# semihkacmaz/CoNFiLD

Measured on AMD Instinct MI355X. Metric: generated fields/sec (256-step sample + CNF decode), Case4 latent, 1/2/4/8 GPU, higher is better.
Workload: dtype f32

## Files before the change

### confild_amd/_lib.py

```python
from __future__ import annotations

import ctypes as C
import os
import threading

_HERE = os.path.dirname(os.path.abspath(__file__))
LIB_PATH = os.path.join(_HERE, "lib", "libconfild_hip.so")
if os.environ.get("CFD_LIB"):
    LIB_PATH = os.path.join(_HERE, "lib", os.path.basename(os.environ["CFD_LIB"]))

_lock = threading.Lock()
_lib = None

c_f32p = C.POINTER(C.c_float)
c_i64p = C.POINTER(C.c_int64)


class CfdError(RuntimeError):
    pass


class UNetCfg(C.Structure):
    _fields_ = [("image_size", C.c_int), ("in_channels", C.c_int), ("model_channels", C.c_int),
                ("out_channels", C.c_int), ("num_res_blocks", C.c_int), ("n_mult", C.c_int),
# ... 35 lines not shown
                                     C.c_void_p, C.c_size_t, C.c_void_p]),
    "cfd_unet_set_tape_mode": (C.c_int, [C.c_void_p, C.c_int]),
    "cfd_sched_create": (C.c_int, [C.c_void_p, C.c_int, C.c_int, C.POINTER(C.c_void_p)]),
    "cfd_sched_destroy": (None, [C.c_void_p]),
    "cfd_sched_step": (C.c_int, [C.c_void_p, C.c_int, C.c_int, C.c_void_p, C.c_void_p, C.c_void_p, C.c_void_p,
                                 C.c_uint64, C.c_uint64, C.c_uint64, C.c_void_p, C.c_void_p, C.c_int64, C.c_int,
                                 C.c_void_p]),
    "cfd_sched_step_known": (C.c_int, [C.c_void_p, C.c_int, C.c_int, C.c_void_p, C.c_void_p, C.c_void_p, C.c_void_p,
                                       C.c_uint64, C.c_uint64, C.c_uint64, C.c_void_p, C.c_void_p, C.c_int64,
                                       C.c_int, C.c_void_p, C.c_int64, C.c_void_p, C.c_int64, C.c_void_p,
                                       C.c_void_p, C.c_uint64, C.c_void_p]),
    "cfd_sched_step_jump": (C.c_int, [C.c_void_p, C.c_int, C.c_int, C.c_void_p, C.c_void_p, C.c_void_p, C.c_void_p,
                                      C.c_uint64, C.c_uint64, C.c_uint64, C.c_void_p, C.c_void_p, C.c_int64,
                                      C.c_int, C.c_void_p, C.c_int64, C.c_void_p, C.c_int64, C.c_void_p,
                                      C.c_void_p, C.c_uint64, C.c_float, C.c_float, C.c_void_p, C.c_uint64,
                                      C.c_void_p]),
    "cfd_sampler_set_jumps": (C.c_int, [C.c_void_p, C.c_void_p]),
    "cfd_sampler_set_known": (C.c_int, [C.c_void_p, C.c_void_p, C.c_int64, C.c_void_p, C.c_int64, C.c_void_p,
                                        C.c_void_p]),
    "cfd_sampler_captures": (C.c_int, [C.c_void_p, C.POINTER(C.c_uint64)]),
    "cfd_dps_latent_residual_workspace_bytes": (C.c_int, [C.c_int64, C.c_int, C.POINTER(C.c_size_t)]),
    "cfd_dps_latent_residual": (C.c_int, [C.c_void_p, C.c_int, C.c_void_p, C.c_void_p, C.c_void_p, C.c_void_p,
                                          C.c_int64, C.c_void_p, C.c_int64, C.c_void_p, C.c_void_p, C.c_void_p,
                                          C.c_int64, C.c_int, C.c_void_p, C.c_size_t, C.c_void_p]),
    "cfd_sampler_create": (C.c_int, [C.c_void_p, C.c_void_p, C.c_int, C.c_int, C.c_int, C.c_int64, C.c_int,
                                     C.c_void_p, C.c_void_p, C.c_int, C.c_int, C.POINTER(C.c_void_p)]),
    "cfd_sampler_destroy": (None, [C.c_void_p]),
    "cfd_sampler_run": (C.c_int, [C.c_void_p, C.c_void_p, C.c_void_p, C.c_int, C.c_int, C.c_uint64, C.c_uint64,
                                  C.c_void_p]),
    "cfd_randn": (C.c_int, [C.c_void_p, C.c_int64, C.c_uint64, C.c_uint64, C.c_uint64, C.c_void_p]),
    "cfd_sine_probe": (C.c_int, [C.c_void_p, C.c_void_p, C.c_int64, C.c_int, C.c_void_p]),
    "cfd_latent_denorm": (C.c_int, [C.c_void_p, C.c_void_p, C.c_int64, C.c_void_p, C.c_void_p, C.c_int64,
                                    C.c_void_p]),
    "cfd_dps_residual": (C.c_int, [C.c_void_p, C.c_int64, C.c_void_p, C.c_void_p, C.c_void_p, C.c_int64, C.c_int,
                                   C.c_void_p]),
    "cfd_dps_latent_grad": (C.c_int, [C.c_void_p, C.c_int, C.c_void_p, C.c_void_p, C.c_void_p, C.c_void_p,
                                      C.c_void_p, C.c_void_p, C.c_int64, C.c_void_p, C.c_void_p, C.c_int64, C.c_int,
                                      C.c_void_p]),
    "cfd_dps_update": (C.c_int, [C.c_void_p, C.c_void_p, C.c_void_p, C.c_float, C.c_void_p, C.c_int64,
                                 C.c_void_p]),
    "cfd_dps_update_known": (C.c_int, [C.c_void_p, C.c_void_p, C.c_void_p, C.c_float, C.c_void_p, C.c_void_p,
                                       C.c_int64, C.c_int, C.c_void_p, C.c_int64, C.c_void_p, C.c_int64, C.c_void_p,
                                       C.c_void_p, C.c_uint64, C.c_uint64, C.c_uint64, C.c_void_p]),
    "cfd_siren_create": (C.c_int, [C.POINTER(SirenCfg), C.c_int, C.POINTER(C.c_void_p)]),
    "cfd_siren_destroy": (None, [C.c_void_p]),
    "cfd_siren_num_params": (C.c_int, [C.c_void_p, C.POINTER(C.c_int)]),
    "cfd_siren_param_info": (C.c_int, [C.c_void_p, C.c_int, C.POINTER(C.c_char_p), C.POINTER(C.c_int),
                                       C.c_int64 * 4]),
    "cfd_siren_set_param": (C.c_int, [C.c_void_p, C.c_char_p, C.c_void_p, C.c_size_t]),
    "cfd_siren_ready": (C.c_int, [C.c_void_p]),
    "cfd_siren_workspace_bytes": (C.c_int, [C.c_void_p, C.c_int, C.POINTER(C.c_size_t)]),
    "cfd_siren_set_compute": (C.c_int, [C.c_void_p, C.c_int]),
    "cfd_siren_get_compute": (C.c_int, [C.c_void_p, C.POINTER(C.c_int)]),
    "cfd_siren_forward": (C.c_int, [C.c_void_p, C.c_void_p, C.c_int64, C.c_void_p, C.c_int, C.c_void_p,
                                    C.c_void_p, C.c_void_p, C.c_void_p, C.c_int64, C.c_void_p, C.c_void_p,
                                    C.c_size_t, C.c_void_p]),
    "cfd_siren_vjp_workspace_bytes": (C.c_int, [C.c_void_p, C.c_int64, C.c_int, C.POINTER(C.c_size_t)]),
    "cfd_siren_tape_forward": (C.c_int, [C.c_void_p, C.c_void_p, C.c_int64, C.c_void_p, C.c_int, C.c_void_p,
                                         C.c_void_p, C.c_void_p, C.c_void_p, C.c_int64, C.c_void_p, C.c_void_p,
                                         C.c_size_t, C.c_void_p]),
    "cfd_siren_tape_vjp": (C.c_int, [C.c_void_p, C.c_void_p, C.c_int64, C.c_int, C.c_void_p, C.c_void_p,
                                     C.c_int64, C.c_void_p, C.c_void_p, C.c_size_t, C.c_void_p]),
    "cfd_siren_dense_plan": (C.c_int, [C.POINTER(SirenCfg), C.c_int64, C.c_int, C.c_size_t, C.c_int, C.c_int,
                                       C.POINTER(C.c_size_t), C.POINTER(C.c_int64), C.POINTER(C.c_int)]),
    "cfd_siren_dense_workspace_bytes": (C.c_int, [C.c_void_p, C.c_int64, C.c_int, C.c_size_t,
                                                  C.POINTER(C.c_size_t)]),
    "cfd_siren_dense_grad": (C.c_int, [C.c_void_p, C.c_void_p, C.c_int64, C.c_void_p, C.c_int, C.c_int, C.c_void_p,
                                       C.c_void_p, C.c_void_p, C.c_void_p, C.c_int64, C.c_void_p, C.c_int,
                                       C.c_void_p, C.c_int, C.c_void_p, C.c_void_p, C.c_void_p, C.c_size_t,
                                       C.c_size_t, C.c_void_p]),
    "cfd_siren_dense_set_form": (C.c_int, [C.c_void_p, C.c_int, C.c_int]),
    "cfd_siren_train_workspace_bytes": (C.c_int, [C.c_void_p, C.c_int64, C.c_int, C.POINTER(C.c_size_t)]),
    "cfd_siren_train_grad": (C.c_int, [C.c_void_p, C.c_void_p, C.c_int64, C.c_void_p, C.c_void_p, C.c_int,
                                       C.c_void_p, C.c_float, C.c_void_p, C.c_void_p, C.c_void_p, C.c_void_p,
                                       C.c_size_t, C.c_void_p]),
    "cfd_unet_param_grad_workspace_bytes": (C.c_int, [C.c_void_p, C.c_int, C.POINTER(C.c_size_t)]),
    "cfd_unet_param_grad": (C.c_int, [C.c_void_p, C.c_void_p, C.c_void_p, C.c_int, C.c_void_p, C.c_size_t,
                                      C.c_void_p, C.c_void_p, C.c_size_t, C.c_void_p]),
    "cfd_eps_mse": (C.c_int, [C.c_void_p, C.c_void_p, C.c_void_p, C.c_void_p, C.c_int64, C.c_int, C.c_float,
                              C.c_void_p, C.c_void_p]),
    "cfd_ema_update": (C.c_int, [C.c_void_p, C.c_void_p, C.c_int64, C.c_double, C.c_void_p]),
    "cfd_q_sample": (C.c_int, [C.c_void_p, C.c_void_p, C.c_void_p, C.c_void_p, C.c_void_p, C.c_int64, C.c_int,
                               C.c_void_p]),
    "cfd_adam_step": (C.c_int, [C.c_void_p, C.c_void_p, C.c_void_p, C.c_void_p, C.c_int64, C.c_double, C.c_double,
                                C.c_double, C.c_double, C.c_double, C.c_int64, C.c_void_p]),
}

EXPORTS = tuple(_SIGS)


def load(path: str = LIB_PATH):
    global _lib
    with _lock:
        if _lib is not None:
            return _lib
        if not os.path.exists(path):
            raise CfdError(f"{path} is missing: build it with `python -c 'import __graft_entry__ as g; g.build()'` "
                           "(or `make -C confild_amd/csrc`)")
        lib = C.CDLL(path)
        for name, (res, args) in _SIGS.items():
            if os.environ.get("CFD_LIB") and not hasattr(lib, name):
                continue
            fn = getattr(lib, name)
            fn.restype = res
            fn.argtypes = args
        _lib = lib
# ... 27 lines not shown
```

### confild_amd/csrc/capi.cpp

```cpp
#include <string>

#include "common.hpp"

namespace cfd {
static thread_local std::string g_last_error;
void set_error(const std::string& msg) { g_last_error = msg; }
}

extern "C" const char* cfd_last_error(void) { return cfd::g_last_error.c_str(); }

extern "C" const char* cfd_version(void) {
    return "libconfild_hip gfx950 r6 (split-f16 / bf16 / fp32 MFMA; native sampler graphs; planned batch; CU-range streams; split-f16 DPS tape; key-chunked attention)";
}
```

### confild_amd/csrc/siren.hpp

```cpp
#pragma once
#include <string>
#include <type_traits>
#include <utility>
#include <vector>

#include "common.hpp"

namespace cfd {

template <int N, class F, int... I>
__device__ __forceinline__ void static_for_impl(F&& f, std::integer_sequence<int, I...>) {
    (f(std::integral_constant<int, I>{}), ...);
}
template <int N, class F>
__device__ __forceinline__ void static_for(F&& f) {
    static_for_impl<N>(f, std::make_integer_sequence<int, N>{});
}

struct SirenArgs {
    const float* w0;
    const float* wimg;
    const float* wout;
    const float* bout;
    const float* film;
    const float* coords;
    const float* xmax;
    const float* xmin;
    const float* ymax;
    const float* ymin;
    float* out;
    const float* wscale;
    const float* wimg_rev;
    const float* wrev;
    int64_t N;
    int64_t ystride;
    int64_t b0;
    int d, c, nh;
    float w0f;
    unsigned long long* stamps;
};
struct SirenTapeArgs {
    const float* w0;
    const float* wimg;
    const float* wimg_t;
    const float* wout;
    const float* bout;
    const float* film;
    const float* coords;
    const float* xmax;
    const float* xmin;
    const float* ymax;
    const float* ymin;
    float* u;
    float* delta;
    float* out;
    const float* gout;
    const float* wimg16;
    const float* wimg16t;
    const float* wscale;
    int64_t P;
    int64_t ystride;
    int Ns, d, c, nh;
    float w0f;
};
unsigned long long* stamps_buf();

template <int NB, int WAVES>
__device__ __forceinline__ void siren_issue_block(const float* __restrict__ wimg, int J, float* dst,
                                                  int wave, int lane) {
    constexpr int BLK = NB * 256;
    const float* src = wimg + (int64_t)__builtin_amdgcn_readfirstlane(J) * BLK;
    for (int piece = wave; piece < NB; piece += WAVES) {
        __builtin_amdgcn_global_load_lds((const void*)(src + piece * 256 + lane * 4),
                                         (__attribute__((address_space(3))) void*)(dst + piece * 256),
                                         16, 0, 0);
    }
}

template <int NB, int WAVES>
__device__ __forceinline__ void siren_issue_block_u(const float* __restrict__ wimg, int J, float* dst,
                                                    int wave, int lane) {
    static_assert(NB % WAVES == 0, "whole pieces per wave");
    constexpr int BLK = NB * 256;
    const float* src = wimg + (int64_t)__builtin_amdgcn_readfirstlane(J) * BLK;
    static_for<NB / WAVES>([&](auto mc) {
        constexpr int m = decltype(mc)::value;
        const int piece = wave + m * WAVES;
        __builtin_amdgcn_global_load_lds((const void*)(src + piece * 256 + lane * 4),
                                         (__attribute__((address_space(3))) void*)(dst + piece * 256), 16, 0, 0);
    });
}

bool siren_split_supported(int NB);
void launch_siren_split(int NB, SirenArgs a, int b, hipStream_t st);
bool siren_split32_supported(int H, int nh);
void launch_siren_split32(int H, SirenArgs a, int b, hipStream_t st);
bool tape_split_supported(int NB);
void launch_tape_split(int NB, const SirenTapeArgs& a, bool bwd, hipStream_t st);
void launch_tape_split_sum(int NB, const SirenTapeArgs& a, int rows, hipStream_t st);

struct SirenParam {
    std::string key;
    std::vector<int64_t> shape;
    bool set = false;
};

}

struct cfd_siren {
    cfd_siren_cfg cfg;
    int device = 0;
    int NB = 0;
    std::vector<cfd::SirenParam> params;
    float* w0 = nullptr;
    float* fbias = nullptr;
    float* V = nullptr;
    float* wimg = nullptr;
    float* wout = nullptr;
    float* bout = nullptr;
    float* wimg_t = nullptr;
    float* wimg16 = nullptr;
    float* wimg16t = nullptr;
    float* wscale = nullptr;
    float* wimg32 = nullptr;
    float* wimg32r = nullptr;
    float* wrev = nullptr;
    int compute = CFD_SIREN_SPLIT_F16;
    int dense_bwd = CFD_DENSE_BWD_SUM;
    int dense_compute = CFD_DENSE_COMPUTE_AUTO;
};

namespace cfd {

int gemm_splits(int K);
void launch_gemm_f32(bool bt, const float* A, int lda, const float* B, int ldb, const float* bias, float* C, int ldc,
                     int M, int N, int K, hipStream_t st, float* part = nullptr);
void film_vectors(const cfd_siren* h, const float* latents, int b, float* film, hipStream_t st);

}
```

### confild_amd/csrc/siren_split.hip

```cpp
#include <cstdint>
#include <cstdlib>
#include <algorithm>

#include "siren.hpp"

typedef _Float16 h8 __attribute__((ext_vector_type(8)));
typedef _Float16 h2 __attribute__((ext_vector_type(2)));
typedef float f2 __attribute__((ext_vector_type(2)));
typedef unsigned u2 __attribute__((ext_vector_type(2)));
typedef unsigned u4 __attribute__((ext_vector_type(4)));

namespace cfd {

struct Frag {
    u4 v;
    __device__ __forceinline__ h8 h() const { return __builtin_bit_cast(h8, v); }
};

__device__ __forceinline__ unsigned pk_f16(float a, float b) {
    return __builtin_bit_cast(unsigned, __builtin_convertvector((f2){a, b}, h2));
}

__device__ __forceinline__ void split8(const float (&x0)[4], const float (&x1)[4], Frag& hi, Frag& lo) {
    unsigned hw[4], lw[4];
#pragma unroll
    for (int w = 0; w < 4; ++w) {
        const float a = w < 2 ? x0[2 * w] : x1[2 * w - 4];
        const float b = w < 2 ? x0[2 * w + 1] : x1[2 * w - 3];
        hw[w] = pk_f16(a, b);
        const f2 hf = __builtin_convertvector(__builtin_bit_cast(h2, hw[w]), f2);
        lw[w] = pk_f16(a - hf.x, b - hf.y);
    }
    hi.v = (u4){hw[0], hw[1], hw[2], hw[3]};
    lo.v = (u4){lw[0], lw[1], lw[2], lw[3]};
    asm volatile("" : "+v"(hi.v), "+v"(lo.v));
}

__device__ __forceinline__ f2 sin2_cw(f2 x) {
    const f2 magic = {12582912.0f, 12582912.0f};
    const f2 t = __builtin_elementwise_fma(x, (f2){0.318309886183790671538f, 0.318309886183790671538f}, magic);
    const f2 q = t - magic;
    f2 r = __builtin_elementwise_fma(q, (f2){-3.140625f, -3.140625f}, x);
    r = __builtin_elementwise_fma(q, (f2){-0.0009670257568359375f, -0.0009670257568359375f}, r);
    r = __builtin_elementwise_fma(q, (f2){-6.2771141529083251953e-07f, -6.2771141529083251953e-07f}, r);
    r = __builtin_elementwise_fma(q, (f2){-1.2154201256553420762e-10f, -1.2154201256553420762e-10f}, r);
    const f2 s = r * r;
    f2 u = (f2){2.6083159809786593541503e-06f, 2.6083159809786593541503e-06f};
    u = __builtin_elementwise_fma(u, s, (f2){-0.0001981069071916863322258f, -0.0001981069071916863322258f});
    u = __builtin_elementwise_fma(u, s, (f2){0.00833307858556509017944336f, 0.00833307858556509017944336f});
    u = __builtin_elementwise_fma(u, s, (f2){-0.166666597127914428710938f, -0.166666597127914428710938f});
    const f2 y = __builtin_elementwise_fma(s, u * r, r);
    const u2 sg = __builtin_bit_cast(u2, t) << 31;
    return __builtin_bit_cast(f2, __builtin_bit_cast(u2, y) + sg);
}

// ... 251 lines not shown
        });
        sines(prev);
        epilogue(std::integral_constant<int, NB - 1>{});
        static_for<NQ>([&](auto qc) {
            constexpr int q = decltype(qc)::value;
#pragma unroll
            for (int c = 0; c < CG; ++c) {
                BH[c][q] = NH[c][q];
                BL[c][q] = NL[c][q];
            }
        });
    }

#pragma unroll
    for (int c = 0; c < CG; ++c) {
        float ov[4];
#pragma unroll
        for (int oc = 0; oc < 4; ++oc) {
            float sum = o[c][oc];
            sum += __shfl_xor(sum, 16);
            sum += __shfl_xor(sum, 32);
            ov[oc] = oc < p.c ? sum + p.bout[oc] : 0.f;
        }
        const int64_t n = n0 + 16 * c;
        if (n < p.N && g < p.c) {
            float v = g == 0 ? ov[0] : g == 1 ? ov[1] : g == 2 ? ov[2] : ov[3];
            if (p.ymax) {
                const int64_t yi = n * p.ystride + g;
                const float hi = p.ymax[yi], lo = p.ymin[yi];
                v = (v + 1.0f) / 2.0f * (hi - lo) + lo;
            }
            p.out[(b * p.N + n) * p.c + g] = v;
        }
    }
}

typedef float f16v __attribute__((ext_vector_type(16)));

__device__ __forceinline__ void split2_mix(float a, float b, unsigned& hi, unsigned& lo) {
    hi = pk_f16(a, b);
    asm("v_fma_mixlo_f16 %0, %1, 1.0, -%2 op_sel_hi:[0,0,1]" : "=&v"(lo) : "v"(a), "v"(hi));
    asm("v_fma_mixhi_f16 %0, %1, 1.0, -%2 op_sel:[0,0,1] op_sel_hi:[0,0,1]" : "+v"(lo) : "v"(b), "v"(hi));
}

__device__ __forceinline__ void split_chunk(const float (&x)[16], int e, Frag& hi, Frag& lo) {
    unsigned hw[4], lw[4];
#pragma unroll
    for (int w = 0; w < 4; ++w) split2_mix(x[8 * e + 2 * w], x[8 * e + 2 * w + 1], hw[w], lw[w]);
    hi.v = (u4){hw[0], hw[1], hw[2], hw[3]};
    lo.v = (u4){lw[0], lw[1], lw[2], lw[3]};
    asm volatile("" : "+v"(hi.v), "+v"(lo.v));
}

template <int NB2, int EXP = 0, int HWSIN = 0>
__global__ __launch_bounds__(256, 1) void siren_split32(SirenArgs p) {
    constexpr int NK = 2 * NB2;
    constexpr int H = 32 * NB2;
    constexpr int BLK = NK * 512;
    constexpr int WAVES = 4, TILE = 128;
    constexpr int NPC = 2 * NK;
    constexpr int PPW = NPC / WAVES;
    constexpr int NKS = NK >= 18 ? 16 : NK - 2;
    extern __shared__ __attribute__((aligned(16))) float smem[];
    const int nh = p.nh;
    float* wbuf = smem;
    float* film = smem + 2 * BLK;
    float* w0s = film + (nh + 1) * H;
    float* wos = w0s + 4 * H;

    const int lane = threadIdx.x & 63;
    const int wave = __builtin_amdgcn_readfirstlane(threadIdx.x >> 6);
    const int h = lane >> 5;
    const int64_t b = p.b0 + blockIdx.y;
    const int64_t n = (int64_t)blockIdx.x * TILE + wave * 32 + (lane & 31);
    CFD_DASSERT(p.d >= 1 && p.d <= 4 && p.c >= 1 && p.c <= 4 && nh >= 1);
#ifdef CFD_STAMPS
    const bool stamped = blockIdx.x % 61 == 0;
    if (stamped) CFD_STAMP(p.stamps, 5, (unsigned)blockIdx.y, 0);
    __builtin_amdgcn_s_waitcnt(0xC07F);
#endif

    {
        const float* fsrc = p.film + b * (int64_t)(nh + 1) * H;
        const int nf = (nh + 1) * H;
        for (int i = threadIdx.x * 4; i < nf; i += 64 * WAVES * 4) {
            const int layer = i / H;
            const float sc = layer == 0 ? 1.0f : HWSIN >= 3 ? p.wrev[layer - 1] : p.wscale[layer - 1];
            *(f4*)(film + i) = *(const f4*)(fsrc + i) * sc;
        }
    }
    for (int f = threadIdx.x; f < H; f += 64 * WAVES) {
        f4 w = {0.f, 0.f, 0.f, 0.f};
        for (int k = 0; k < p.d; ++k) w[k] = p.w0[f * p.d + k];
        *(f4*)(w0s + 4 * f) = w;
    }
    for (int i = threadIdx.x; i < 4 * H; i += 64 * WAVES) wos[i] = i < p.c * H ? p.wout[i] : 0.f;
    float cn[4];
    {
        const int64_t nc = n < p.N ? n : p.N - 1;
#pragma unroll
        for (int k = 0; k < 4; ++k) {
            float v = 0.f;
            if (k < p.d) {
                v = p.coords[nc * p.d + k];
                if (p.xmax) v = (v - p.xmin[k]) / (p.xmax[k] - p.xmin[k]) * 2.0f - 1.0f;
            }
            cn[k] = v;
        }
    }
    __syncthreads();
    const int nblocks = nh * NB2;
    const __amdgpu_buffer_rsrc_t wrsrc =
        __builtin_amdgcn_make_buffer_rsrc((void*)p.wimg, 0, nblocks * (BLK * 4), 0x00020000);
    siren_issue_block<NPC, WAVES>(p.wimg, 0, wbuf, wave, lane);

    Frag BH[NK], BL[NK], NH[NK], NL[NK];
    float o[4] = {0.f, 0.f, 0.f, 0.f};

    static_for<NB2>([&](auto Jc) {
        constexpr int J = decltype(Jc)::value;
        float x[16];
#pragma unroll
        for (int qq = 0; qq < 4; ++qq) {
            const f4 fv = *(const f4*)(film + 32 * J + 8 * qq + 4 * h);
#pragma unroll
            for (int r = 0; r < 4; ++r) {
                const f4 w = *(const f4*)(w0s + 4 * (32 * J + 8 * qq + 4 * h + r));
                float a = cn[0] * w[0];
#pragma unroll
                for (int k = 1; k < 4; ++k)
                    if (k < p.d) a = fmaf(cn[k], w[k], a);
                x[4 * qq + r] = hidden_sine<HWSIN >= 2 ? 2 : HWSIN>(p.w0f * (a + fv[r]));
            }
        }
        split_chunk(x, 0, NH[2 * J], NL[2 * J]);
        split_chunk(x, 1, NH[2 * J + 1], NL[2 * J + 1]);
    });

    static_assert(NB2 % 2 == 0, "static ring slots need an even block count");
    int J = 0;
    f16v prev;
    float mprev = 0.f;
    float x[16];
    for (int layer = 1; layer <= nh; ++layer) {
        const bool last = layer == nh;
        const float m = HWSIN >= 3 ? p.wrev[nh + layer - 1] : p.w0f / p.wscale[layer - 1];
        auto outsum = [&](int jp, int e) __attribute__((always_inline)) {
            const int f = 32 * jp + 8 * e + 4 * h;
#pragma unroll
            for (int oc = 0; oc < 4; ++oc) {
                const f4 w = *(const f4*)(wos + oc * H + f);
#pragma unroll
                for (int r = 0; r < 4; ++r) o[oc] = fmaf(w[r], x[4 * e + r], o[oc]);
            }
        };
        static_for<NB2>([&](auto jc) {
            constexpr int j = decltype(jc)::value;
            constexpr int jp = j == 0 ? NB2 - 1 : j - 1;
            const float me = j == 0 ? mprev : m;
            const bool live = j > 0 || layer > 1;
            float* nxt = wbuf + ((j & 1) ^ 1) * BLK;
            const float* wb = wbuf + (j & 1) * BLK;
            const int soff = __builtin_amdgcn_readfirstlane(min(J + 1, nblocks - 1)) * (BLK * 4);
            f16v a;
#pragma unroll
            for (int qq = 0; qq < 4; ++qq) {
                const f4 f = *(const f4*)(film + layer * H + 32 * j + 8 * qq + 4 * h);
#pragma unroll
                for (int r = 0; r < 4; ++r) a[4 * qq + r] = f[r];
            }
            h8 FH = *(const h8*)(wb + lane * 4);
            h8 FL = *(const h8*)(wb + 256 + lane * 4);
            static_for<NK>([&](auto kc) {
                constexpr int k = decltype(kc)::value;
                h8 FH1 = FH, FL1 = FL;
                if constexpr (k + 1 < NK && !(EXP & 4)) {
                    FH1 = *(const h8*)(wb + (k + 1) * 512 + lane * 4);
                    FL1 = *(const h8*)(wb + (k + 1) * 512 + 256 + lane * 4);
                }
                if constexpr (k < PPW && !(EXP & 1)) {
                    const int piece = wave + WAVES * k;
                    __builtin_amdgcn_raw_ptr_buffer_load_lds(
                        wrsrc, (__attribute__((address_space(3))) void*)(nxt + piece * 256), 16, lane * 16,
                        soff + piece * 1024, 0, 0);
                }
                if constexpr (j == 0) {
                    a = __builtin_amdgcn_mfma_f32_32x32x16_f16(FL, NH[k].h(), a, 0, 0, 0);
                    a = __builtin_amdgcn_mfma_f32_32x32x16_f16(FH, NL[k].h(), a, 0, 0, 0);
                    a = __builtin_amdgcn_mfma_f32_32x32x16_f16(FH, NH[k].h(), a, 0, 0, 0);
                    BH[k] = NH[k];
                    BL[k] = NL[k];
                    asm volatile("" : "+a"(BH[k].v), "+a"(BL[k].v));
                } else {
                    a = __builtin_amdgcn_mfma_f32_32x32x16_f16(FL, BH[k].h(), a, 0, 0, 0);
                    a = __builtin_amdgcn_mfma_f32_32x32x16_f16(FH, BL[k].h(), a, 0, 0, 0);
                    a = __builtin_amdgcn_mfma_f32_32x32x16_f16(FH, BH[k].h(), a, 0, 0, 0);
                }
                if constexpr (k < NKS) {
#pragma unroll
                    for (int v = 16 * k / NKS; v < 16 * (k + 1) / NKS; ++v) {
                        x[v] = (EXP & 2) ? prev[v] * me : hidden_sine<HWSIN>(prev[v] * me);
                        asm volatile("" : "+v"(x[v]));
                    }
                }
                constexpr int KE = NK >= 18 ? 16 : NKS - 1;
                if constexpr (k == KE || k == (NK >= 18 ? 17 : KE)) {
                    constexpr bool both = NK < 18;
                    constexpr int e0 = (NK >= 18 && k == 17) ? 1 : 0;
                    if (live) {
#pragma unroll
                        for (int e = e0; e < (both ? 2 : e0 + 1); ++e)
                            split_chunk(x, e, NH[2 * jp + e], NL[2 * jp + e]);
                        if (j > 0 && last) {
#pragma unroll
                            for (int e = 2 * e0; e < (both ? 4 : 2 * e0 + 2); ++e) outsum(jp, e);
                        }
                    }
                }
                __builtin_amdgcn_sched_barrier(0);
                FH = FH1;
                FL = FL1;
            });
            prev = a;
            if constexpr (!(EXP & 1)) {
                __builtin_amdgcn_s_waitcnt(vmcnt_imm(0));
                asm volatile("s_barrier" ::: "memory");
            }
            ++J;
        });
        mprev = m;
    }
#pragma unroll
    for (int v = 0; v < 16; ++v) x[v] = hidden_sine<HWSIN>(prev[v] * mprev);
    {
        const int f0 = 32 * (NB2 - 1) + 4 * h;
#pragma unroll
        for (int e = 0; e < 4; ++e)
#pragma unroll
            for (int oc = 0; oc < 4; ++oc) {
                const f4 w = *(const f4*)(wos + oc * H + f0 + 8 * e);
#pragma unroll
                for (int r = 0; r < 4; ++r) o[oc] = fmaf(w[r], x[4 * e + r], o[oc]);
            }
    }

    float ov[4];
#pragma unroll
    for (int oc = 0; oc < 4; ++oc) {
        const float sum = o[oc] + __shfl_xor(o[oc], 32);
        ov[oc] = oc < p.c ? sum + p.bout[oc] : 0.f;
    }
    if (n < p.N) {
#pragma unroll
        for (int i = 0; i < 2; ++i) {
            const int oc = 2 * h + i;
            if (oc < p.c) {
                float v = ov[oc];
                if (p.ymax) {
                    const int64_t yi = n * p.ystride + oc;
                    const float hi = p.ymax[yi], lo = p.ymin[yi];
                    v = (v + 1.0f) / 2.0f * (hi - lo) + lo;
                }
                p.out[(b * p.N + n) * p.c + oc] = v;
            }
        }
    }
#ifdef CFD_STAMPS
    if (stamped) CFD_STAMP(p.stamps, 5, (unsigned)blockIdx.y, 4);
#endif
}

namespace {

template <int NB, int RING, int CG, int RB = 1, bool NOSYNC = false, bool PKSIN = true>
void launch_ring(SirenArgs a, int b, hipStream_t st) {
    constexpr int H = NB * 16;
    constexpr int WAVES = CG == 1 ? 8 : 4;
    const size_t lds = sizeof(float) * ((size_t)RING * RB * NB * 256 + (size_t)(a.nh + 1) * H + 8 * H);
    const void* fn = (const void*)siren_fused_split<NB, WAVES, RING, CG, RB, NOSYNC, PKSIN>;
    CFD_REQUIRE(lds <= 160 * 1024, CFD_EARG, "SIREN too deep for the split-f16 decoder's LDS staging");
    CFD_HIP(hipFuncSetAttribute(fn, hipFuncAttributeMaxDynamicSharedMemorySize, (int)lds));
    const int64_t tiles = ceil_div(a.N, 16 * CG * WAVES);
    CFD_REQUIRE(tiles <= 0x7fffffff, CFD_EARG, "too many coordinates for one launch");
    for (int64_t b0 = 0; b0 < b; b0 += 65535) {
        a.b0 = b0;
        const int nb = (int)std::min<int64_t>(65535, b - b0);
        hipLaunchKernelGGL((siren_fused_split<NB, WAVES, RING, CG, RB, NOSYNC, PKSIN>), dim3((unsigned)tiles, nb),
                           dim3(64 * WAVES), lds, st, a);
        check_launch("siren_fused_split");
    }
}

template <int NB>
void launch_nb(SirenArgs a, int b, hipStream_t st) {
    launch_ring<NB, 2, 1, 1>(a, b, st);
}
}

template <int NB2, int EXP = 0, int HWSIN = 0>
void launch_split32(SirenArgs a, int b, hipStream_t st) {
    constexpr int H = NB2 * 32;
    const size_t lds = sizeof(float) * ((size_t)2 * 2 * NB2 * 512 + (size_t)(a.nh + 1) * H + 8 * H);
    const void* fn = (const void*)siren_split32<NB2, EXP, HWSIN>;
    CFD_REQUIRE((int64_t)a.nh * H * H * 4 < 0x7fffffffLL, CFD_EARG, "weight image beyond the 2 GiB buffer range");
    CFD_REQUIRE(lds <= 160 * 1024, CFD_EARG, "SIREN too deep for the split-f16 decoder's LDS staging");
    CFD_HIP(hipFuncSetAttribute(fn, hipFuncAttributeMaxDynamicSharedMemorySize, (int)lds));
    const int64_t tiles = ceil_div(a.N, 128);
    CFD_REQUIRE(tiles <= 0x7fffffff, CFD_EARG, "too many coordinates for one launch");
    for (int64_t b0 = 0; b0 < b; b0 += 65535) {
        a.b0 = b0;
        const int nb = (int)std::min<int64_t>(65535, b - b0);
        hipLaunchKernelGGL((siren_split32<NB2, EXP, HWSIN>), dim3((unsigned)tiles, nb), dim3(256), lds, st, a);
        check_launch("siren_split32");
    }
}

bool siren_split32_supported(int H, int nh) {
    const size_t film = (size_t)(nh + 1) * H + 8 * (size_t)H;
    return (H == 64 || H == 128 || H == 256 || H == 384) &&
           sizeof(float) * ((size_t)4 * (H / 32) * 512 + film) <= 160 * 1024;
}

void launch_siren_split32(int H, SirenArgs a, int b, hipStream_t st) {
    CFD_REQUIRE(a.wimg_rev && a.wrev, CFD_EARG, "split32 revolution image not set");
    a.wimg = a.wimg_rev;
    switch (H) {
        case 64: return launch_split32<2, 0, 4>(a, b, st);
        case 128: return launch_split32<4, 0, 4>(a, b, st);
        case 256: return launch_split32<8, 0, 4>(a, b, st);
        case 384: return launch_split32<12, 0, 4>(a, b, st);
        default: throw Error{CFD_EARG, "32x32 split-f16 SIREN needs hidden_features in {64, 128, 256, 384}"};
    }
}

bool siren_split_supported(int NB) {
    switch (NB) {
        case 2: case 4: case 6: case 8: case 12: case 16: case 24: return true;
        default: return false;
    }
}

void launch_siren_split(int NB, SirenArgs a, int b, hipStream_t st) {
    switch (NB) {
        case 2: return launch_nb<2>(a, b, st);
        case 4: return launch_nb<4>(a, b, st);
        case 6: return launch_nb<6>(a, b, st);
        case 8: return launch_nb<8>(a, b, st);
        case 12: return launch_nb<12>(a, b, st);
        case 16: return launch_nb<16>(a, b, st);
        case 24: return launch_nb<24>(a, b, st);
        default: throw Error{CFD_EARG, "split-f16 SIREN needs hidden_features = 32*{1,2,3,4,6,8,12,16}"};
    }
}

template <int NB, int KS, int RING>
__global__ __launch_bounds__(64 * KS) void siren_tape_fwd_split(SirenTapeArgs p) {
    constexpr int H = NB * 16, BLK = NB * 256, QW = NB / KS, QC = QW / 2;
    static_assert(QW % 2 == 0 && (RING == 2 || RING == 3), "K9t: an even block count per wave");
    extern __shared__ __attribute__((aligned(16))) float smem[];
    float* wbuf = smem;
    float* red = smem + RING * BLK;
    const int lane = threadIdx.x & 63;
    const int wave = __builtin_amdgcn_readfirstlane(threadIdx.x >> 6);
    const int g = lane >> 4, j16 = lane & 15;
    const int64_t n = (int64_t)blockIdx.x * 16 + j16;
    const int64_t nc = n < p.P ? n : p.P - 1;
// ... 439 lines not shown
```

### include/confild.h

```cpp
#ifndef CONFILD_H
#define CONFILD_H

#include <stddef.h>
#include <stdint.h>

#ifdef __cplusplus
extern "C" {
#endif

enum { CFD_OK = 0, CFD_EARG = 1, CFD_EHIP = 2, CFD_EKEY = 3, CFD_ESHAPE = 4, CFD_ESTATE = 5 };

const char* cfd_last_error(void);
const char* cfd_version(void);

typedef struct cfd_unet cfd_unet;

typedef struct {
    int image_size;
    int in_channels;
    int model_channels;
    int out_channels;
    int num_res_blocks;
    int n_mult;
    int channel_mult[8];
// ... 61 lines not shown
int  cfd_device_cu_count(int device, int* n_cu);
int  cfd_stream_create_cu_range(int device, int first_cu, int n_cu, void** stream);
int  cfd_stream_destroy(void* stream);
int  cfd_sampler_run(cfd_sampler* sp, const float* x_in, float* x_out, int k0, int k1, uint64_t seed,
                     uint64_t offset, void* stream);
int  cfd_sampler_set_known(cfd_sampler* sp, const float* known, int64_t known_bstride, const float* mask,
                           int64_t mask_bstride, const float* table, void* stream);
int  cfd_sampler_captures(const cfd_sampler* sp, uint64_t* n);
int  cfd_sampler_set_jumps(cfd_sampler* sp, const float* host_jtab);
int  cfd_randn(float* out, int64_t n, uint64_t seed, uint64_t counter, uint64_t offset, void* stream);
int  cfd_sine_probe(const float* x, float* y, int64_t n, int which, void* stream);
int  cfd_latent_denorm(const float* x, float* y, int64_t n, const float* vmax, const float* vmin,
                       int64_t period, void* stream);

int  cfd_dps_residual(const float* y, int64_t y_batch_stride, const float* A, float* g_A, float* norm,
                      int64_t n_per_sample, int B, void* stream);
int  cfd_dps_latent_grad(const cfd_sched* s, int clip, const float* x, const float* eps, const int64_t* t,
                         const float* g_z, const float* vmax, const float* vmin, int64_t period,
                         float* d_eps, float* g_direct, int64_t n_per_sample, int B, void* stream);
int  cfd_dps_update(const float* sample, const float* g_direct, const float* g_unet, float scale,
                    float* x_out, int64_t n, void* stream);
int  cfd_dps_update_known(const float* sample, const float* g_direct, const float* g_unet, float scale,
                          float* x_out, const int64_t* t, int64_t n_per_sample, int B, const float* known,
                          int64_t known_bstride, const float* mask, int64_t mask_bstride, const float* table,
                          const float* noise2, uint64_t seed, uint64_t counter2, uint64_t offset, void* stream);
int  cfd_dps_latent_residual_workspace_bytes(int64_t n_per_sample, int B, size_t* bytes);
int  cfd_dps_latent_residual(const cfd_sched* s, int clip, const float* x, const float* eps, const int64_t* t,
                             const float* y, int64_t y_bstride, const float* mask, int64_t mask_bstride,
                             float* norm, float* d_eps, float* g_direct, int64_t n_per_sample, int B,
                             void* workspace, size_t ws_bytes, void* stream);

typedef struct cfd_siren cfd_siren;

typedef struct {
    int in_coord_features;
    int in_latent_features;
    int out_features;
    int num_hidden_layers;
    int hidden_features;
    float w0;
} cfd_siren_cfg;

int  cfd_siren_create(const cfd_siren_cfg* cfg, int device, cfd_siren** out);
void cfd_siren_destroy(cfd_siren* h);
int  cfd_siren_num_params(const cfd_siren* h, int* n);
int  cfd_siren_param_info(const cfd_siren* h, int idx, const char** key, int* ndim, int64_t shape[4]);
int  cfd_siren_set_param(cfd_siren* h, const char* key, const float* host_data, size_t n);
int  cfd_siren_ready(const cfd_siren* h);
int  cfd_siren_workspace_bytes(const cfd_siren* h, int b, size_t* bytes);
#define CFD_SIREN_F32       0
#define CFD_SIREN_SPLIT_F16 1
int  cfd_siren_set_compute(cfd_siren* h, int compute);
int  cfd_siren_get_compute(const cfd_siren* h, int* compute);
int  cfd_siren_forward(cfd_siren* h, const float* coords, int64_t N, const float* latents, int b,
                       const float* xmax, const float* xmin,
                       const float* ymax, const float* ymin, int64_t y_stride,
                       float* out, void* workspace, size_t ws_bytes, void* stream);

int  cfd_siren_vjp_workspace_bytes(const cfd_siren* h, int64_t Ns, int R, size_t* bytes);
int  cfd_siren_tape_forward(cfd_siren* h, const float* coords, int64_t Ns, const float* latents, int R,
                            const float* xmax, const float* xmin,
                            const float* ymax, const float* ymin, int64_t y_stride,
                            float* out, void* workspace, size_t ws_bytes, void* stream);
int  cfd_siren_tape_vjp(cfd_siren* h, const float* g_out, int64_t Ns, int R,
                        const float* ymax, const float* ymin, int64_t y_stride,
                        float* g_latents, void* workspace, size_t ws_bytes, void* stream);

#define CFD_DENSE_SLAB 64
#define CFD_DENSE_DEFAULT_BUDGET ((size_t)1 << 30)
int  cfd_siren_dense_plan(const cfd_siren_cfg* cfg, int64_t N, int R, size_t budget, int bwd_form,
                          int compute_form, size_t* bytes, int64_t* chunk_points, int* block_rows);
int  cfd_siren_dense_workspace_bytes(const cfd_siren* h, int64_t N, int R, size_t budget, size_t* bytes);
int  cfd_siren_dense_grad(cfd_siren* h, const float* coords, int64_t N,
                          const float* latents, int R, int rows_per_sample,
                          const float* xmax, const float* xmin,
                          const float* ymax, const float* ymin, int64_t y_stride,
                          const float* y, int y_rows,
                          const float* mask, int mask_rows,
                          float* g_latents, float* norm,
                          void* workspace, size_t ws_bytes, size_t budget, void* stream);
#define CFD_DENSE_BWD_SUM   0
#define CFD_DENSE_BWD_DELTA 1
#define CFD_DENSE_COMPUTE_AUTO  0
#define CFD_DENSE_COMPUTE_F32   1
int  cfd_siren_dense_set_form(cfd_siren* h, int bwd_form, int compute_form);

int  cfd_siren_train_workspace_bytes(const cfd_siren* h, int64_t N, int R, size_t* bytes);
int  cfd_siren_train_grad(cfd_siren* h, const float* coords, int64_t N, const float* latents,
                          const int64_t* rows, int R, const float* target, float scale,
                          float* grad, float* grad_latents, float* sse,
                          void* workspace, size_t ws_bytes, void* stream);
int  cfd_unet_param_grad_workspace_bytes(const cfd_unet* h, int B, size_t* bytes);
int  cfd_unet_param_grad(cfd_unet* h, const float* x, const float* d_eps, int B, const void* tape,
                         size_t tape_bytes, float* grad, void* workspace, size_t ws_bytes, void* stream);
int  cfd_eps_mse(const float* eps, const float* noise, const float* weights, float* d_eps,
                 int64_t n_per_sample, int B, float scale, float* sse, void* stream);
int  cfd_ema_update(float* target, const float* source, int64_t n, double rate, void* stream);
int  cfd_q_sample(const float* x0, const float* noise, const float* coef_a, const float* coef_s, float* x_t,
                  int64_t n_per_sample, int B, void* stream);
int  cfd_adam_step(float* param, const float* grad, float* exp_avg, float* exp_avg_sq, int64_t n,
                   double lr, double beta1, double beta2, double eps, double weight_decay, int64_t step,
                   void* stream);

#ifdef __cplusplus
}
#endif
// ... 2 lines not shown
```

Baseline: 3.919.

## Make split32 SIREN decoder persistent over multiple coordinate tiles per workgroup

```diff
diff --git a/confild_amd/_lib.py b/confild_amd/_lib.py
--- a/confild_amd/_lib.py
+++ b/confild_amd/_lib.py
@@ -111,6 +111,8 @@
     "cfd_siren_workspace_bytes": (C.c_int, [C.c_void_p, C.c_int, C.POINTER(C.c_size_t)]),
     "cfd_siren_set_compute": (C.c_int, [C.c_void_p, C.c_int]),
     "cfd_siren_get_compute": (C.c_int, [C.c_void_p, C.POINTER(C.c_int)]),
+    "cfd_siren_set_tiles_per_wg": (C.c_int, [C.c_int]),
+    "cfd_siren_tiles_per_wg": (C.c_int, [C.c_int64, C.c_int64, C.c_int, C.POINTER(C.c_int)]),
     "cfd_siren_forward": (C.c_int, [C.c_void_p, C.c_void_p, C.c_int64, C.c_void_p, C.c_int, C.c_void_p,
                                     C.c_void_p, C.c_void_p, C.c_void_p, C.c_int64, C.c_void_p, C.c_void_p,
                                     C.c_size_t, C.c_void_p]),
diff --git a/confild_amd/csrc/capi.cpp b/confild_amd/csrc/capi.cpp
--- a/confild_amd/csrc/capi.cpp
+++ b/confild_amd/csrc/capi.cpp
@@ -1,6 +1,6 @@
 #include <string>
 
-#include "common.hpp"
+#include "siren.hpp"
 
 namespace cfd {
 static thread_local std::string g_last_error;
@@ -12,3 +12,18 @@
 extern "C" const char* cfd_version(void) {
     return "libconfild_hip gfx950 r6 (split-f16 / bf16 / fp32 MFMA; native sampler graphs; planned batch; CU-range streams; split-f16 DPS tape; key-chunked attention)";
 }
+
+extern "C" int cfd_siren_set_tiles_per_wg(int tiles) {
+    return cfd::guard([&] {
+        CFD_REQUIRE(tiles >= 0 && tiles <= 4096, CFD_EARG, "tiles per workgroup outside [0, 4096]");
+        cfd::siren_set_tiles_per_wg(tiles);
+    });
+}
+
+extern "C" int cfd_siren_tiles_per_wg(int64_t rows, int64_t n_coords, int n_cu, int* tiles) {
+    return cfd::guard([&] {
+        CFD_REQUIRE(tiles && rows >= 1 && n_coords >= 1, CFD_EARG, "bad argument");
+        if (n_cu <= 0) CFD_REQUIRE(cfd_device_cu_count(0, &n_cu) == 0, CFD_EARG, "no device");
+        *tiles = cfd::siren_tiles_per_wg(rows, n_coords, n_cu);
+    });
+}
diff --git a/confild_amd/csrc/siren.hpp b/confild_amd/csrc/siren.hpp
--- a/confild_amd/csrc/siren.hpp
+++ b/confild_amd/csrc/siren.hpp
@@ -38,6 +38,8 @@
     int d, c, nh;
     float w0f;
     unsigned long long* stamps;
+    int64_t tiles;
+    int tpw;
 };
 struct SirenTapeArgs {
     const float* w0;
@@ -95,6 +97,8 @@
 void launch_siren_split(int NB, SirenArgs a, int b, hipStream_t st);
 bool siren_split32_supported(int H, int nh);
 void launch_siren_split32(int H, SirenArgs a, int b, hipStream_t st);
+int siren_tiles_per_wg(int64_t rows, int64_t n_coords, int cus);
+void siren_set_tiles_per_wg(int tpw);
 bool tape_split_supported(int NB);
 void launch_tape_split(int NB, const SirenTapeArgs& a, bool bwd, hipStream_t st);
 void launch_tape_split_sum(int NB, const SirenTapeArgs& a, int rows, hipStream_t st);
diff --git a/confild_amd/csrc/siren_split.hip b/confild_amd/csrc/siren_split.hip
--- a/confild_amd/csrc/siren_split.hip
+++ b/confild_amd/csrc/siren_split.hip
@@ -1,6 +1,7 @@
 #include <cstdint>
 #include <cstdlib>
 #include <algorithm>
+#include <atomic>
 
 #include "siren.hpp"
 
@@ -358,7 +359,7 @@
     asm volatile("" : "+v"(hi.v), "+v"(lo.v));
 }
 
-template <int NB2, int EXP = 0, int HWSIN = 0>
+template <int NB2, int EXP = 0, int HWSIN = 0, int D = 0>
 __global__ __launch_bounds__(256, 1) void siren_split32(SirenArgs p) {
     constexpr int NK = 2 * NB2;
     constexpr int H = 32 * NB2;
@@ -377,15 +378,22 @@
     const int lane = threadIdx.x & 63;
     const int wave = __builtin_amdgcn_readfirstlane(threadIdx.x >> 6);
     const int h = lane >> 5;
+    const int d = D ? D : p.d;
     const int64_t b = p.b0 + blockIdx.y;
-    const int64_t n = (int64_t)blockIdx.x * TILE + wave * 32 + (lane & 31);
+    const int64_t tile0 = (int64_t)blockIdx.x * p.tpw;
+    const int ntile = (int)min((int64_t)p.tpw, p.tiles - tile0);
     CFD_DASSERT(p.d >= 1 && p.d <= 4 && p.c >= 1 && p.c <= 4 && nh >= 1);
+    CFD_DASSERT((D == 0 || D == p.d) && p.tpw >= 1 && ntile >= 1 && p.tiles == (p.N + TILE - 1) / TILE);
 #ifdef CFD_STAMPS
     const bool stamped = blockIdx.x % 61 == 0;
     if (stamped) CFD_STAMP(p.stamps, 5, (unsigned)blockIdx.y, 0);
     __builtin_amdgcn_s_waitcnt(0xC07F);
 #endif
 
+    const int nblocks = nh * NB2;
+    const __amdgpu_buffer_rsrc_t wrsrc =
+        __builtin_amdgcn_make_buffer_rsrc((void*)p.wimg, 0, nblocks * (BLK * 4), 0x00020000);
+    siren_issue_block<NPC, WAVES>(p.wimg, 0, wbuf, wave, lane);
     {
         const float* fsrc = p.film + b * (int64_t)(nh + 1) * H;
         const int nf = (nh + 1) * H;
@@ -397,179 +405,214 @@
     }
     for (int f = threadIdx.x; f < H; f += 64 * WAVES) {
         f4 w = {0.f, 0.f, 0.f, 0.f};
-        for (int k = 0; k < p.d; ++k) w[k] = p.w0[f * p.d + k];
+        for (int k = 0; k < d; ++k) w[k] = p.w0[f * d + k];
         *(f4*)(w0s + 4 * f) = w;
     }
     for (int i = threadIdx.x; i < 4 * H; i += 64 * WAVES) wos[i] = i < p.c * H ? p.wout[i] : 0.f;
-    float cn[4];
-    {
-        const int64_t nc = n < p.N ? n : p.N - 1;
-#pragma unroll
-        for (int k = 0; k < 4; ++k) {
-            float v = 0.f;
-            if (k < p.d) {
-                v = p.coords[nc * p.d + k];
-                if (p.xmax) v = (v - p.xmin[k]) / (p.xmax[k] - p.xmin[k]) * 2.0f - 1.0f;
-            }
-            cn[k] = v;
-        }
-    }
+    auto args = [&]() __attribute__((always_inline)) {
+        auto kp = (const __attribute__((address_space(4))) SirenArgs*)__builtin_amdgcn_kernarg_segment_ptr();
+        asm volatile("" : "+s"(kp));
+        return kp;
+    };
+    auto load_coords = [&](int t, float (&cr)[4]) __attribute__((always_inline)) {
+        const auto q = args();
+        const int64_t nt = ((int64_t)blockIdx.x * q->tpw + t) * TILE + wave * 32 + (lane & 31);
+        const int64_t nc = nt < q->N ? nt : q->N - 1;
+        const int dd = D ? D : q->d;
+        CFD_DASSERT(t >= 0 && t < ntile && nc >= 0);
+        const float* cp = q->coords + nc * dd;
+#pragma unroll
+        for (int k = 0; k < 4; ++k) cr[k] = k < dd ? cp[k] : 0.f;
+    };
+    float cr[4];
+    load_coords(0, cr);
+    if constexpr (!(EXP & 1)) __builtin_amdgcn_s_waitcnt(vmcnt_imm(0));
     __syncthreads();
-    const int nblocks = nh * NB2;
-    const __amdgpu_buffer_rsrc_t wrsrc =
-        __builtin_amdgcn_make_buffer_rsrc((void*)p.wimg, 0, nblocks * (BLK * 4), 0x00020000);
-    siren_issue_block<NPC, WAVES>(p.wimg, 0, wbuf, wave, lane);
 
     Frag BH[NK], BL[NK], NH[NK], NL[NK];
-    float o[4] = {0.f, 0.f, 0.f, 0.f};
-
-    static_for<NB2>([&](auto Jc) {
-        constexpr int J = decltype(Jc)::value;
-        float x[16];
-#pragma unroll
-        for (int qq = 0; qq < 4; ++qq) {
-            const f4 fv = *(const f4*)(film + 32 * J + 8 * qq + 4 * h);
-#pragma unroll
-            for (int r = 0; r < 4; ++r) {
-                const f4 w = *(const f4*)(w0s + 4 * (32 * J + 8 * qq + 4 * h + r));
-                float a = cn[0] * w[0];
-#pragma unroll
-                for (int k = 1; k < 4; ++k)
-                    if (k < p.d) a = fmaf(cn[k], w[k], a);
-                x[4 * qq + r] = hidden_sine<HWSIN >= 2 ? 2 : HWSIN>(p.w0f * (a + fv[r]));
-            }
-        }
-        split_chunk(x, 0, NH[2 * J], NL[2 * J]);
-        split_chunk(x, 1, NH[2 * J + 1], NL[2 * J + 1]);
-    });
-
-    static_assert(NB2 % 2 == 0, "static ring slots need an even block count");
-    int J = 0;
+    float x[16];
     f16v prev;
     float mprev = 0.f;
-    float x[16];
-    for (int layer = 1; layer <= nh; ++layer) {
-        const bool last = layer == nh;
-        const float m = HWSIN >= 3 ? p.wrev[nh + layer - 1] : p.w0f / p.wscale[layer - 1];
-        auto outsum = [&](int jp, int e) __attribute__((always_inline)) {
-            const int f = 32 * jp + 8 * e + 4 * h;
-#pragma unroll
-            for (int oc = 0; oc < 4; ++oc) {
-                const f4 w = *(const f4*)(wos + oc * H + f);
-#pragma unroll
-                for (int r = 0; r < 4; ++r) o[oc] = fmaf(w[r], x[4 * e + r], o[oc]);
-            }
-        };
-        static_for<NB2>([&](auto jc) {
-            constexpr int j = decltype(jc)::value;
-            constexpr int jp = j == 0 ? NB2 - 1 : j - 1;
-            const float me = j == 0 ? mprev : m;
-            const bool live = j > 0 || layer > 1;
-            float* nxt = wbuf + ((j & 1) ^ 1) * BLK;
-            const float* wb = wbuf + (j & 1) * BLK;
-            const int soff = __builtin_amdgcn_readfirstlane(min(J + 1, nblocks - 1)) * (BLK * 4);
-            f16v a;
+
+    for (int t = 0; t < ntile; ++t) {
+        const bool ltile = t == ntile - 1;
+        float o[4] = {0.f, 0.f, 0.f, 0.f};
+        float cn[4];
+        const auto q0 = args();
+        const int dd = D ? D : q0->d;
+        const float w0f = q0->w0f;
+        {
+            const float *xmax = q0->xmax, *xmin = q0->xmin;
+#pragma unroll
+            for (int k = 0; k < 4; ++k) {
+                float v = cr[k];
+                if (k < dd && xmax) v = (v - xmin[k]) / (xmax[k] - xmin[k]) * 2.0f - 1.0f;
+                cn[k] = v;
+            }
+        }
+
+        static_for<NB2>([&](auto Jc) {
+            constexpr int J = decltype(Jc)::value;
+            float x0[16];
 #pragma unroll
             for (int qq = 0; qq < 4; ++qq) {
-                const f4 f = *(const f4*)(film + layer * H + 32 * j + 8 * qq + 4 * h);
-#pragma unroll
-                for (int r = 0; r < 4; ++r) a[4 * qq + r] = f[r];
-            }
-            h8 FH = *(const h8*)(wb + lane * 4);
-            h8 FL = *(const h8*)(wb + 256 + lane * 4);
-            static_for<NK>([&](auto kc) {
-                constexpr int k = decltype(kc)::value;
-                h8 FH1 = FH, FL1 = FL;
-                if constexpr (k + 1 < NK && !(EXP & 4)) {
-                    FH1 = *(const h8*)(wb + (k + 1) * 512 + lane * 4);
-                    FL1 = *(const h8*)(wb + (k + 1) * 512 + 256 + lane * 4);
-                }
-                if constexpr (k < PPW && !(EXP & 1)) {
-                    const int piece = wave + WAVES * k;
-                    __builtin_amdgcn_raw_ptr_buffer_load_lds(
-                        wrsrc, (__attribute__((address_space(3))) void*)(nxt + piece * 256), 16, lane * 16,
-                        soff + piece * 1024, 0, 0);
-                }
-                if constexpr (j == 0) {
-                    a = __builtin_amdgcn_mfma_f32_32x32x16_f16(FL, NH[k].h(), a, 0, 0, 0);
-                    a = __builtin_amdgcn_mfma_f32_32x32x16_f16(FH, NL[k].h(), a, 0, 0, 0);
-                    a = __builtin_amdgcn_mfma_f32_32x32x16_f16(FH, NH[k].h(), a, 0, 0, 0);
-                    BH[k] = NH[k];
-                    BL[k] = NL[k];
-                    asm volatile("" : "+a"(BH[k].v), "+a"(BL[k].v));
-                } else {
-                    a = __builtin_amdgcn_mfma_f32_32x32x16_f16(FL, BH[k].h(), a, 0, 0, 0);
-                    a = __builtin_amdgcn_mfma_f32_32x32x16_f16(FH, BL[k].h(), a, 0, 0, 0);
-                    a = __builtin_amdgcn_mfma_f32_32x32x16_f16(FH, BH[k].h(), a, 0, 0, 0);
-                }
-                if constexpr (k < NKS) {
-#pragma unroll
-                    for (int v = 16 * k / NKS; v < 16 * (k + 1) / NKS; ++v) {
-                        x[v] = (EXP & 2) ? prev[v] * me : hidden_sine<HWSIN>(prev[v] * me);
-                        asm volatile("" : "+v"(x[v]));
-                    }
-                }
-                constexpr int KE = NK >= 18 ? 16 : NKS - 1;
-                if constexpr (k == KE || k == (NK >= 18 ? 17 : KE)) {
-                    constexpr bool both = NK < 18;
-                    constexpr int e0 = (NK >= 18 && k == 17) ? 1 : 0;
-                    if (live) {
-#pragma unroll
-                        for (int e = e0; e < (both ? 2 : e0 + 1); ++e)
-                            split_chunk(x, e, NH[2 * jp + e], NL[2 * jp + e]);
-                        if (j > 0 && last) {
-#pragma unroll
-                            for (int e = 2 * e0; e < (both ? 4 : 2 * e0 + 2); ++e) outsum(jp, e);
+                const f4 fv = *(const f4*)(film + 32 * J + 8 * qq + 4 * h);
+#pragma unroll
+                for (int r = 0; r < 4; ++r) {
+                    const f4 w = *(const f4*)(w0s + 4 * (32 * J + 8 * qq + 4 * h + r));
+                    float a = cn[0] * w[0];
+#pragma unroll
+                    for (int k = 1; k < 4; ++k) {
+                        if constexpr (D != 0) {
+                            if (k < D) a = fmaf(cn[k], w[k], a);
+                        } else {
+                            if (k < dd) a = fmaf(cn[k], w[k], a);
                         }
                     }
-                }
-                __builtin_amdgcn_sched_barrier(0);
-                FH = FH1;
-                FL = FL1;
+                    x0[4 * qq + r] = hidden_sine<HWSIN >= 2 ? 2 : HWSIN>(w0f * (a + fv[r]));
+                }
+            }
+            split_chunk(x0, 0, NH[2 * J], NL[2 * J]);
+            split_chunk(x0, 1, NH[2 * J + 1], NL[2 * J + 1]);
+        });
+#ifdef CFD_STAMPS
+        if (stamped) CFD_STAMP(p.stamps, 5, (unsigned)blockIdx.y, 8 * t + 1);
+#endif
+
+        static_assert(NB2 % 2 == 0, "static ring slots need an even block count");
+        int J = 0;
+        for (int layer = 1; layer <= nh; ++layer) {
+            const bool last = layer == nh;
+            const float m = HWSIN >= 3 ? p.wrev[nh + layer - 1] : p.w0f / p.wscale[layer - 1];
+            auto outsum = [&](int jp, int e) __attribute__((always_inline)) {
+                const int f = 32 * jp + 8 * e + 4 * h;
+#pragma unroll
+                for (int oc = 0; oc < 4; ++oc) {
+                    const f4 w = *(const f4*)(wos + oc * H + f);
+#pragma unroll
+                    for (int r = 0; r < 4; ++r) o[oc] = fmaf(w[r], x[4 * e + r], o[oc]);
+                }
+            };
+            static_for<NB2>([&](auto jc) {
+                constexpr int j = decltype(jc)::value;
+                constexpr int jp = j == 0 ? NB2 - 1 : j - 1;
+                const float me = j == 0 ? mprev : m;
+                const bool live = j > 0 || layer > 1;
+                float* nxt = wbuf + ((j & 1) ^ 1) * BLK;
+                const float* wb = wbuf + (j & 1) * BLK;
+                const int jn = J + 1 < nblocks ? J + 1 : ltile ? nblocks - 1 : 0;
+                const int soff = __builtin_amdgcn_readfirstlane(jn) * (BLK * 4);
+                f16v a;
+#pragma unroll
+                for (int qq = 0; qq < 4; ++qq) {
+                    const f4 f = *(const f4*)(film + layer * H + 32 * j + 8 * qq + 4 * h);
+#pragma unroll
+                    for (int r = 0; r < 4; ++r) a[4 * qq + r] = f[r];
+                }
+                h8 FH = *(const h8*)(wb + lane * 4);
+                h8 FL = *(const h8*)(wb + 256 + lane * 4);
+                static_for<NK>([&](auto kc) {
+                    constexpr int k = decltype(kc)::value;
+                    h8 FH1 = FH, FL1 = FL;
+                    if constexpr (k + 1 < NK && !(EXP & 4)) {
+                        FH1 = *(const h8*)(wb + (k + 1) * 512 + lane * 4);
+                        FL1 = *(const h8*)(wb + (k + 1) * 512 + 256 + lane * 4);
+                    }
+                    if constexpr (k < PPW && !(EXP & 1)) {
+                        const int piece = wave + WAVES * k;
+                        __builtin_amdgcn_raw_ptr_buffer_load_lds(
+                            wrsrc, (__attribute__((address_space(3))) void*)(nxt + piece * 256), 16, lane * 16,
+                            soff + piece * 1024, 0, 0);
+                    }
+                    if constexpr (j == 0) {
+                        a = __builtin_amdgcn_mfma_f32_32x32x16_f16(FL, NH[k].h(), a, 0, 0, 0);
+                        a = __builtin_amdgcn_mfma_f32_32x32x16_f16(FH, NL[k].h(), a, 0, 0, 0);
+                        a = __builtin_amdgcn_mfma_f32_32x32x16_f16(FH, NH[k].h(), a, 0, 0, 0);
+                        BH[k] = NH[k];
+                        BL[k] = NL[k];
+                        asm volatile("" : "+a"(BH[k].v), "+a"(BL[k].v));
+                    } else {
+                        a = __builtin_amdgcn_mfma_f32_32x32x16_f16(FL, BH[k].h(), a, 0, 0, 0);
+                        a = __builtin_amdgcn_mfma_f32_32x32x16_f16(FH, BL[k].h(), a, 0, 0, 0);
+                        a = __builtin_amdgcn_mfma_f32_32x32x16_f16(FH, BH[k].h(), a, 0, 0, 0);
+                    }
+                    if constexpr (k < NKS) {
+#pragma unroll
+                        for (int v = 16 * k / NKS; v < 16 * (k + 1) / NKS; ++v) {
+                            x[v] = (EXP & 2) ? prev[v] * me : hidden_sine<HWSIN>(prev[v] * me);
+                            asm volatile("" : "+v"(x[v]));
+                        }
+                    }
+                    constexpr int KE = NK >= 18 ? 16 : NKS - 1;
+                    if constexpr (k == KE || k == (NK >= 18 ? 17 : KE)) {
+                        constexpr bool both = NK < 18;
+                        constexpr int e0 = (NK >= 18 && k == 17) ? 1 : 0;
+                        if (live) {
+#pragma unroll
+                            for (int e = e0; e < (both ? 2 : e0 + 1); ++e)
+                                split_chunk(x, e, NH[2 * jp + e], NL[2 * jp + e]);
+                            if (j > 0 && last) {
+#pragma unroll
+                                for (int e = 2 * e0; e < (both ? 4 : 2 * e0 + 2); ++e) outsum(jp, e);
+                            }
+                        }
+                    }
+                    __builtin_amdgcn_sched_barrier(0);
+                    FH = FH1;
+                    FL = FL1;
+                });
+                prev = a;
+                if constexpr (!(EXP & 1)) {
+                    __builtin_amdgcn_s_waitcnt(vmcnt_imm(0));
+                    asm volatile("s_barrier" ::: "memory");
+                }
+                ++J;
             });
-            prev = a;
-            if constexpr (!(EXP & 1)) {
-                __builtin_amdgcn_s_waitcnt(vmcnt_imm(0));
-                asm volatile("s_barrier" ::: "memory");
-            }
-            ++J;
-        });
-        mprev = m;
-    }
-#pragma unroll
-    for (int v = 0; v < 16; ++v) x[v] = hidden_sine<HWSIN>(prev[v] * mprev);
-    {
-        const int f0 = 32 * (NB2 - 1) + 4 * h;
-#pragma unroll
-        for (int e = 0; e < 4; ++e)
-#pragma unroll
-            for (int oc = 0; oc < 4; ++oc) {
-                const f4 w = *(const f4*)(wos + oc * H + f0 + 8 * e);
-#pragma unroll
-                for (int r = 0; r < 4; ++r) o[oc] = fmaf(w[r], x[4 * e + r], o[oc]);
-            }
-    }
-
-    float ov[4];
-#pragma unroll
-    for (int oc = 0; oc < 4; ++oc) {
-        const float sum = o[oc] + __shfl_xor(o[oc], 32);
-        ov[oc] = oc < p.c ? sum + p.bout[oc] : 0.f;
-    }
-    if (n < p.N) {
-#pragma unroll
-        for (int i = 0; i < 2; ++i) {
-            const int oc = 2 * h + i;
-            if (oc < p.c) {
-                float v = ov[oc];
-                if (p.ymax) {
-                    const int64_t yi = n * p.ystride + oc;
-                    const float hi = p.ymax[yi], lo = p.ymin[yi];
-                    v = (v + 1.0f) / 2.0f * (hi - lo) + lo;
-                }
-                p.out[(b * p.N + n) * p.c + oc] = v;
-            }
-        }
+            mprev = m;
+        }
+#ifdef CFD_STAMPS
+        if (stamped) CFD_STAMP(p.stamps, 5, (unsigned)blockIdx.y, 8 * t + 2);
+#endif
+        if (!ltile) load_coords(t + 1, cr);
+        const int64_t n = ((int64_t)blockIdx.x * args()->tpw + t) * TILE + wave * 32 + (lane & 31);
+#pragma unroll
+        for (int v = 0; v < 16; ++v) x[v] = hidden_sine<HWSIN>(prev[v] * mprev);
+        {
+            const int f0 = 32 * (NB2 - 1) + 4 * h;
+#pragma unroll
+            for (int e = 0; e < 4; ++e)
+#pragma unroll
+                for (int oc = 0; oc < 4; ++oc) {
+                    const f4 w = *(const f4*)(wos + oc * H + f0 + 8 * e);
+#pragma unroll
+                    for (int r = 0; r < 4; ++r) o[oc] = fmaf(w[r], x[4 * e + r], o[oc]);
+                }
+        }
+
+        float ov[4];
+#pragma unroll
+        for (int oc = 0; oc < 4; ++oc) {
+            const float sum = o[oc] + __shfl_xor(o[oc], 32);
+            ov[oc] = oc < p.c ? sum + p.bout[oc] : 0.f;
+        }
+        if (n < p.N) {
+#pragma unroll
+            for (int i = 0; i < 2; ++i) {
+                const int oc = 2 * h + i;
+                if (oc < p.c) {
+                    float v = ov[oc];
+                    if (p.ymax) {
+                        const int64_t yi = n * p.ystride + oc;
+                        const float hi = p.ymax[yi], lo = p.ymin[yi];
+                        v = (v + 1.0f) / 2.0f * (hi - lo) + lo;
+                    }
+                    p.out[(b * p.N + n) * p.c + oc] = v;
+                }
+            }
+        }
+#ifdef CFD_STAMPS
+        if (stamped) CFD_STAMP(p.stamps, 5, (unsigned)blockIdx.y, 8 * t + 3);
+#endif
     }
 #ifdef CFD_STAMPS
     if (stamped) CFD_STAMP(p.stamps, 5, (unsigned)blockIdx.y, 4);
@@ -603,21 +646,57 @@
 }
 }
 
-template <int NB2, int EXP = 0, int HWSIN = 0>
-void launch_split32(SirenArgs a, int b, hipStream_t st) {
+namespace {
+std::atomic<int> g_tiles_per_wg{0};
+
+int device_cus() {
+    static std::atomic<int> cus[64];
+    int dev = 0, n = 0;
+    CFD_HIP(hipGetDevice(&dev));
+    if (dev >= 0 && dev < 64 && (n = cus[dev].load()) > 0) return n;
+    CFD_HIP(hipDeviceGetAttribute(&n, hipDeviceAttributeMultiprocessorCount, dev));
+    if (dev >= 0 && dev < 64) cus[dev].store(n);
+    return n;
+}
+}
+
+void siren_set_tiles_per_wg(int tpw) { g_tiles_per_wg.store(tpw); }
+
+int siren_tiles_per_wg(int64_t rows, int64_t n_coords, int cus) {
+    if (const int f = g_tiles_per_wg.load(); f > 0) return f;
+    const int64_t tiles = ceil_div(n_coords, (int64_t)128);
+    for (int t = 16; t > 1; t /= 2)
+        if (rows * ceil_div(tiles, (int64_t)t) >= 16 * (int64_t)cus) return t;
+    return 1;
+}
+
+template <int NB2, int EXP = 0, int HWSIN = 0, int D = 0>
+void launch_split32_d(SirenArgs a, int b, hipStream_t st) {
     constexpr int H = NB2 * 32;
     const size_t lds = sizeof(float) * ((size_t)2 * 2 * NB2 * 512 + (size_t)(a.nh + 1) * H + 8 * H);
-    const void* fn = (const void*)siren_split32<NB2, EXP, HWSIN>;
+    const void* fn = (const void*)siren_split32<NB2, EXP, HWSIN, D>;
     CFD_REQUIRE((int64_t)a.nh * H * H * 4 < 0x7fffffffLL, CFD_EARG, "weight image beyond the 2 GiB buffer range");
     CFD_REQUIRE(lds <= 160 * 1024, CFD_EARG, "SIREN too deep for the split-f16 decoder's LDS staging");
     CFD_HIP(hipFuncSetAttribute(fn, hipFuncAttributeMaxDynamicSharedMemorySize, (int)lds));
-    const int64_t tiles = ceil_div(a.N, 128);
-    CFD_REQUIRE(tiles <= 0x7fffffff, CFD_EARG, "too many coordinates for one launch");
+    a.tiles = ceil_div(a.N, (int64_t)128);
+    CFD_REQUIRE(a.tiles <= 0x7fffffff, CFD_EARG, "too many coordinates for one launch");
+    a.tpw = siren_tiles_per_wg(b, a.N, device_cus());
+    const int64_t groups = ceil_div(a.tiles, (int64_t)a.tpw);
     for (int64_t b0 = 0; b0 < b; b0 += 65535) {
         a.b0 = b0;
         const int nb = (int)std::min<int64_t>(65535, b - b0);
-        hipLaunchKernelGGL((siren_split32<NB2, EXP, HWSIN>), dim3((unsigned)tiles, nb), dim3(256), lds, st, a);
+        hipLaunchKernelGGL((siren_split32<NB2, EXP, HWSIN, D>), dim3((unsigned)groups, nb), dim3(256), lds, st, a);
         check_launch("siren_split32");
+    }
+}
+
+template <int NB2, int EXP = 0, int HWSIN = 0>
+void launch_split32(SirenArgs a, int b, hipStream_t st) {
+    CFD_REQUIRE(a.d >= 1 && a.d <= 4, CFD_EARG, "the split-f16 decoder takes 1 to 4 coordinate features");
+    switch (a.d) {
+        case 2: return launch_split32_d<NB2, EXP, HWSIN, 2>(a, b, st);
+        case 3: return launch_split32_d<NB2, EXP, HWSIN, 3>(a, b, st);
+        default: return launch_split32_d<NB2, EXP, HWSIN, 0>(a, b, st);
     }
 }
 
diff --git a/include/confild.h b/include/confild.h
--- a/include/confild.h
+++ b/include/confild.h
@@ -137,6 +137,8 @@
 #define CFD_SIREN_SPLIT_F16 1
 int  cfd_siren_set_compute(cfd_siren* h, int compute);
 int  cfd_siren_get_compute(const cfd_siren* h, int* compute);
+int  cfd_siren_set_tiles_per_wg(int tiles);
+int  cfd_siren_tiles_per_wg(int64_t rows, int64_t n_coords, int n_cu, int* tiles);
 int  cfd_siren_forward(cfd_siren* h, const float* coords, int64_t N, const float* latents, int b,
                        const float* xmax, const float* xmin,
                        const float* ymax, const float* ymin, int64_t y_stride,
```

After: 3.953, median of 6. No clear change (+0.8%).
